# hanruihua/RDA-planner

Measured on AMD Instinct MI355X. Metric: MPC steps/sec (ADMM early stop or iter_num cap: see residuals), T=20, N_obs=200, higher is better.
Workload: dtype f64; 1 GPU; north-star: acker rectangle robot, T=20, N_obs=200 static seeded polygons, E=4, iter_num=4, iter_threshold=0.2, ro1=200; parallelism=single GPU

## Files before the change

rda_planner_amd/csrc/lammuz_device.h:

```cpp
#pragma once
#include <hip/hip_runtime.h>
#include <math.h>

#pragma clang fp contract(on)

namespace lmz {

constexpr int EMAX = 8;
constexpr int RMAX = 8;
constexpr double SIGN_TOL = 1e-12;

struct WaveLDS {
    double A[EMAX][2];
    double b[EMAX];
    double q[EMAX];
    double M[EMAX][2];
    unsigned char lamc[40];
    double vtx[28][2];
    int npv, nlv;
};
struct RobotLDS {
    double G[RMAX][2];
    double h[RMAX];
    unsigned char muc[40]; int nmv;
// ... 314 lines not shown
    if (norm2) {
        if (lane == 0) { W.lamc[0] = 1; W.lamc[1] = 2; W.lamc[2] = 0; W.npv = 0; W.nlv = 3; }
    } else {
        bool vp = false; double vx = 0, vy = 0;
        if (lane < E * (E - 1) / 2) {
            int i1, i2; decode_pair(lane, E, i1, i2);
            const double a00 = W.A[i1][0], a01 = W.A[i1][1], a10 = W.A[i2][0], a11 = W.A[i2][1];
            const double det = a00 * a11 - a01 * a10;
            if (det != 0 && det * det > 1e-24 * (a00 * a00 + a01 * a01) * (a10 * a10 + a11 * a11)) {
                const double wx = W.b[i1] * a11 - a01 * W.b[i2], wy = a00 * W.b[i2] - W.b[i1] * a10, sg = det > 0 ? 1.0 : -1.0, ad = fabs(det);
                vp = true;
                for (int k = 0; k < E; ++k) {
                    const double ak0 = W.A[k][0], ak1 = W.A[k][1], bk = W.b[k];
                    const double viol = sg * (ak0 * wx + ak1 * wy - bk * det);
                    if (viol > 1e-9 * (ad + fabs(bk) * ad + fabs(ak0 * wx) + fabs(ak1 * wy))) vp = false;
                }
                vx = wx / det; vy = wy / det;
            }
        }
        const bool vs = lane < E && (W.A[lane < E ? lane : 0][0] != 0 || W.A[lane < E ? lane : 0][1] != 0);
        const unsigned long long bp = __ballot(vp), bs = __ballot(vs), below = (1ull << lane) - 1;
        const int npv = __popcll(bp), nsv = __popcll(bs);
        if (vp) { const int k = __popcll(bp & below); W.lamc[k] = (unsigned char)(1 + E + lane); W.vtx[k][0] = vx; W.vtx[k][1] = vy; }
        if (vs) W.lamc[npv + __popcll(bs & below)] = (unsigned char)(1 + lane);
        if (lane == 0) { W.lamc[npv + nsv] = 0; W.npv = npv; W.nlv = npv + nsv + 1; }
    }
}

__device__ __forceinline__ void wave_sync()
{
    __builtin_amdgcn_fence(__ATOMIC_RELEASE, "workgroup");
    __builtin_amdgcn_wave_barrier();
    __builtin_amdgcn_fence(__ATOMIC_ACQUIRE, "workgroup");
}

__device__ __forceinline__ void prepare_wave(WaveLDS &W, const Params &P, int lane)
{
    pose_products(W, P, lane);
    build_lists(W, P.E, P.norm2, lane);
    wave_sync();
}

__device__ __forceinline__ void solve_wave(WaveLDS &W, const RobotLDS &Rb, const Params &P, int lane, Sol &best)
{
    const int nm = 1 + P.R + P.R * (P.R - 1) / 2;
    const int nlv = W.nlv, nmv = Rb.nmv;
    const int half = nlv * nmv;
    best.cost = INFINITY; best.id = 0x7fffffff;
    best.m = 0; best.H0 = 0; best.H1 = 0; best.i1 = best.i2 = best.j1 = best.j2 = -1;
    best.l1 = best.l2 = best.g1 = best.g2 = 0;
    long long tprev = P.prof ? clock64() : 0;
    auto mark = [&](int k) { if (P.prof && lane == 0) { long long now = clock64(); P.prof[k] += now - tprev; tprev = now; } };
    for (int ic = 0; ic < 2; ++ic) {
        int itn = 0;
        for (int c = lane; c < half; c += 64) {
            const int ilx = c / nmv, il = W.lamc[ilx], im = Rb.muc[c - ilx * nmv];
            Sol s;
            if (eval_candidate(W, Rb, P, il, im, ic, s)) {
                s.id = 2 * (il * nm + im) + ic;
                if (s.cost < best.cost || (s.cost == best.cost && s.id < best.id)) best = s;
            }
            mark(1 + 2 * ic + (itn < 1 ? itn : 1)); ++itn;
        }
        double bc = best.cost; int bid = best.id;
#pragma unroll
        for (int off = 32; off >= 1; off >>= 1) {
            double oc = __shfl_xor(bc, off, 64); int oid = __shfl_xor(bid, off, 64);
            if (oc < bc || (oc == bc && oid < bid)) { bc = oc; bid = oid; }
        }
        unsigned long long win = __ballot(best.id == bid);
        int src = __ffsll((long long)win) - 1;
        best.cost = __shfl(best.cost, src, 64); best.id = bid;
        best.m = __shfl(best.m, src, 64); best.H0 = __shfl(best.H0, src, 64); best.H1 = __shfl(best.H1, src, 64);
        best.i1 = __shfl(best.i1, src, 64); best.i2 = __shfl(best.i2, src, 64);
        best.j1 = __shfl(best.j1, src, 64); best.j2 = __shfl(best.j2, src, 64);
        best.l1 = __shfl(best.l1, src, 64); best.l2 = __shfl(best.l2, src, 64);
        best.g1 = __shfl(best.g1, src, 64); best.g2 = __shfl(best.g2, src, 64);
        mark(5 + ic);
        if (best.m >= 0) break;
        if (ic == 0) best.cost += 0.5 * best.m * best.m;
    }
}

template <int CTRL> __device__ __forceinline__ double dpp_mov_f64(double v)
{
    int lo = __builtin_amdgcn_update_dpp(0, __double2loint(v), CTRL, 0xf, 0xf, false);
    int hi = __builtin_amdgcn_update_dpp(0, __double2hiint(v), CTRL, 0xf, 0xf, false);
    return __hiloint2double(hi, lo);
}
template <int CTRL> __device__ __forceinline__ double dpp_mov0_f64(double v)
{
    int lo = __builtin_amdgcn_update_dpp(0, __double2loint(v), CTRL, 0xf, 0xf, true);
    int hi = __builtin_amdgcn_update_dpp(0, __double2hiint(v), CTRL, 0xf, 0xf, true);
    return __hiloint2double(hi, lo);
}
__device__ __forceinline__ double wave_max(double v)
{
    double o;
    o = dpp_mov_f64<0xB1>(v); v = o > v ? o : v;
    o = dpp_mov_f64<0x4E>(v); v = o > v ? o : v;
    o = dpp_mov_f64<0x141>(v); v = o > v ? o : v;
    o = dpp_mov_f64<0x140>(v); v = o > v ? o : v;
    o = __shfl_xor(v, 16, 64); v = o > v ? o : v;
    o = __shfl_xor(v, 32, 64); v = o > v ? o : v;
    return v;
}

__device__ __forceinline__ double row_max(double v)
{
    double o;
    o = dpp_mov_f64<0xB1>(v); v = o > v ? o : v;
    o = dpp_mov_f64<0x4E>(v); v = o > v ? o : v;
    o = dpp_mov_f64<0x141>(v); v = o > v ? o : v;
    o = dpp_mov_f64<0x140>(v); v = o > v ? o : v;
    return v;
}
template <int GW> struct Grp {
    static __device__ __forceinline__ unsigned long long ballot(bool p, int lane)
    {
        const unsigned long long b = __ballot(p);
        if (GW == 64) return b;
        return (b >> (lane & 48)) & 0xffffull;
    }
    static __device__ __forceinline__ double max(double v) { return GW == 64 ? wave_max(v) : row_max(v); }
    template <typename Tv> static __device__ __forceinline__ Tv bcast(Tv v, int src) { return __shfl(v, src, GW); }
};

__device__ __forceinline__ int support_neighbour(int c, int n, const unsigned char *cand, int ncand, int k)
{
    if (c == 0) { int seen = 0; for (int q = 0; q < ncand; ++q) { const int v = cand[q]; if (v >= 1 && v <= n) { if (seen == k) return v; ++seen; } } return -1; }
    if (c <= n) {
        if (k == 0) return 0;
        int seen = 1;
        for (int q = 0; q < ncand; ++q) {
            const int v = cand[q];
            if (v > n) { int a, b; decode_pair(v - 1 - n, n, a, b); if (a == c - 1 || b == c - 1) { if (seen == k) return v; ++seen; } }
        }
        return -1;
    }
    int a, b; decode_pair(c - 1 - n, n, a, b);
    return k == 0 ? 1 + a : (k == 1 ? 1 + b : -1);
}

template <int GW> __device__ __forceinline__ bool warm_circle(const WaveLDS &W, const RobotLDS &Rb, const Params &P, int wlane, int hint, Sol &best)
{
    const int lane = wlane & (GW - 1), R = P.R, E = P.E, nm0 = 1 + R + R * (R - 1) / 2;
    if (hint < 0) return false;
    const int il = hint / nm0, im = hint - il * nm0;
    if (il > 2) return false;
    auto certify = [&]() -> bool {
        const double na = best.i1 >= 0 ? hypot(best.l1, best.l2) : 0.0;
        if (na > 1.0 + 1e-12) return false;
        if ((best.j1 >= 0 && !(best.g1 > 1e-12)) || (best.j2 >= 0 && !(best.g2 > 1e-12))) return false;
        const double phim = (best.m < 0 ? best.m : 0.0) - P.delta;
        const double dvx = P.px - W.b[0], dvy = P.py - W.b[1], l0 = W.b[2];
        const double ut0 = P.cs * dvx + P.sn * dvy, ut1 = -P.sn * dvx + P.cs * dvy;
        const double at0 = P.cs * best.l1 + P.sn * best.l2, at1 = -P.sn * best.l1 + P.cs * best.l2;
        const double g0 = phim * ut0 + P.ro2 * best.H0, g1 = phim * ut1 + P.ro2 * best.H1, ck = phim * l0;
        const double gs = fabs(phim) * (hypot(ut0, ut1) + fabs(l0)) + P.ro2 * hypot(best.H0, best.H1);
        bool pass;
        if (!(na > 0)) pass = hypot(g0, g1) < ck * (1.0 - 1e-6);
        else {
            const double gr0 = g0 + ck * at0 / na, gr1 = g1 + ck * at1 / na;
            if (na < 1.0 - 1e-6) pass = na > 1e-6 && hypot(gr0, gr1) <= 1e-7 * gs;
            else { const double nu = -(gr0 * at0 + gr1 * at1), tz = gr1 * at0 - gr0 * at1; pass = na >= 1.0 - 1e-12 && nu > 1e-6 * gs && fabs(tz) <= 1e-7 * gs; }
        }
// ... 279 lines not shown
```

rda_planner_amd/csrc/rda_hip.hip:

```cpp
#include <hip/hip_runtime.h>
#include <cfloat>
#include <climits>
#include <cstdio>
#include <cstdlib>
#include <cstring>
#include <vector>
#include <chrono>
#include <memory>
#include <dlfcn.h>
#include "../../include/rda_hip.h"
#include "host_buf.h"
#include "lammuz_device.h"
#include "lammuz_cp_device.h"
#include "lammuz_ip_device.h"
#include "su_device.h"
#include "scene_device.h"
#include "lidar_device.h"
#include "track_device.h"
#include "rollout_device.h"

#define HIPCHK(x) do { hipError_t e_ = (x); if (e_ != hipSuccess) { \
    fprintf(stderr, "librda_hip: %s failed: %s (%s:%d)\n", #x, hipGetErrorString(e_), __FILE__, __LINE__); return RDA_ERR_HIP; } } while (0)

struct Ctrl {
// ... 444 lines not shown
    const size_t o = drow(d, n, t + 1), zi = drow(d, n, t);
    P.xi0 = d.xi[2 * o]; P.xi1 = d.xi[2 * o + 1];
    const double zeta = d.zeta[zi], dbar = d.dis[t];
    P.kappa0 = zeta - dbar; P.ro2 = d.c.ro2; P.delta = d.c.delta;
    lmz::Sol best;
    double prev = 0.0;
    if (lane < E) prev = d.lam[o * E + lane];
    else if (lane < E + R) prev = d.mu[o * R + lane - E];
    bool bad = !isfinite(P.px + P.py + P.cs + P.sn + P.xi0 + P.xi1 + P.kappa0);
    if (lane < 2 * E) bad = bad || !isfinite(W.A[lane >> 1][lane & 1]);
    if (lane < E) bad = bad || !isfinite(W.b[lane]);
    bad = __ballot(bad) != 0;
    if (bad) {
        if (lane < 2 * E) W.A[lane >> 1][lane & 1] = 0;
        if (lane < E) W.b[lane] = 0;
        P.px = P.py = P.sn = P.xi0 = P.xi1 = P.kappa0 = 0; P.cs = 1;
        lmz::wave_sync();
    }
    lmz::pose_products(W, P, lane);
    {
        const size_t oc = (size_t)n * d.nt + (d.nt > 1 ? t + 1 : 0);
        if (lane < d.oc_ls) W.lamc[lane] = d.oc_lamc[oc * d.oc_ls + lane];
        if (lane < d.oc_vs) (&W.vtx[0][0])[lane] = d.oc_vtx[oc * d.oc_vs + lane];
        if (lane == 0) { W.npv = d.oc_cnt[2 * oc]; W.nlv = d.oc_cnt[2 * oc + 1]; }
    }
    lmz::wave_sync();
    const int hpar = d.ctrl->hint_par & 1;
    if (!d.warm || !lmz::solve_wave_warm<64>(W, rb, P, lane, hint_read(d, hpar, n, t, it == 0), best)) lmz::solve_wave(W, rb, P, lane, best);
    if (lane == 0) hint_write(d, hpar, n, t, best.id >> 1);
    if (d.centre) lmz::central_normal_wave<64>(W, rb, P, lane, best);
    bad = bad || !(isfinite(best.cost) && isfinite(best.m) && isfinite(best.H0) && isfinite(best.H1));
    const int k = t * d.Nloc + nl;
    if (bad) {
        if (lane == 0) {
            store_row(d, k, failed_row(d, k));
            hint_write(d, hpar, n, t, -1);
            atomicAdd(&d.ctrl->lmz_fail, 1);
        }
        return;
    }
    const double znew = (d.c.accelerated ? 0.5 : 1.0) * (best.m > 0 ? best.m : 0.0);
    double res = 0;
    if (lane < E) {
        double v = lmz::lam_of(best, P.norm2, lane);
        res = (v - prev) * (v - prev); d.lam[o * E + lane] = v;
    } else if (lane < E + R) {
        int j = lane - E;
        double v = lmz::mu_of(best, j);
        res = (v - prev) * (v - prev); d.mu[o * R + j] = v;
    } else if (lane == E + R) {
        double old = d.z[zi];
        res = (znew - old) * (znew - old); d.z[zi] = znew;
    }
#pragma unroll
    for (int off = 32; off >= 1; off >>= 1) res += __shfl_xor(res, off, 64);
    if (lane == 0) {
        double ax = 0, ay = 0, bl = 0, mh = 0, gx = 0, gy = 0;
        for (int i = 0; i < E; ++i) {
            double v = lmz::lam_of(best, P.norm2, i);
            ax += v * W.A[i][0]; ay += v * W.A[i][1]; bl += v * W.b[i];
        }
        for (int j = 0; j < R; ++j) {
            double v = lmz::mu_of(best, j);
            mh += v * rb.h[j]; gx += v * rb.G[j][0]; gy += v * rb.G[j][1];
        }
        const double hx = gx + P.cs * ax + P.sn * ay, hy = gy - P.sn * ax + P.cs * ay;
        const double xin0 = P.xi0 + hx, xin1 = P.xi1 + hy;
        d.xi[2 * o] = xin0; d.xi[2 * o + 1] = xin1;
        const double im = ax * P.px + ay * P.py - bl - mh;
        const double zetan = zeta + im - dbar - znew;
        d.zeta[zi] = zetan;
        RowOut ro; ro.ax = ax; ro.ay = ay; ro.bl = bl; ro.c3 = mh + znew - zetan; ro.c4 = gx + xin0; ro.c5 = gy + xin1;
        ro.res = res; ro.hh = hx * hx + hy * hy;
        store_row(d, k, ro);
    }
}

__global__ __launch_bounds__(256) void k_lammuz(Dev d, int it) { lammuz_body(d, blockIdx.x, it); }

#ifdef RDA_LMZ_CLK
__device__ unsigned long long *g_lmz_clk = nullptr;
constexpr int LMZ_CLK_WORDS = 32;
__device__ int *g_lmz_faillog = nullptr;
#endif
template <int MODE = 0, bool CW = false> __device__ __forceinline__ void lammuz_body_rows(const Dev &d, const int block, const int nblocks, const int it, const Fin &fin)
{
#pragma clang fp contract(on)
    constexpr int WPB = GS / 4;
    constexpr bool LANES = CW;
    __shared__ lmz::WaveLDS wl[GS];
    __shared__ lmz::RobotLDS rb;
    __shared__ double rowv[MODE == 0 ? GS : 1][6];
    const int T = d.c.T, E = d.c.E, R = d.c.R;
#ifdef RDA_LMZ_CLK
    long long clk_prev = clock64(); const long long clk_in = clk_prev; bool clk_enum = false; const unsigned long long clk_wall_in = (unsigned long long)wall_clock64();
    unsigned long long *const clk_slot = g_lmz_clk ? g_lmz_clk + LMZ_CLK_WORDS * (size_t)(block * (GS / 4) + (threadIdx.x >> 6)) : nullptr;
    long long clk_sub = clk_prev;
#define LMZ_CLK(k) do { if (MODE == 0) { const long long now_ = clock64(); if (clk_slot && (threadIdx.x & 63) == 0) clk_slot[k] += (unsigned long long)(now_ - clk_prev); clk_prev = now_; clk_sub = now_; } } while (0)
#define LMZ_SUB(k) do { if (MODE == 0) { const long long now_ = clock64(); if (clk_slot && (threadIdx.x & 63) == 0) clk_slot[16 + (k)] += (unsigned long long)(now_ - clk_sub); clk_sub = now_; } } while (0)
#else
#define LMZ_CLK(k) do { } while (0)
#define LMZ_SUB(k) do { } while (0)
#endif
    int tb = 0, jb = 0;
    if (MODE != 2) { block_of(d, block, tb, jb); if (tb < 0) return; }
    const int lane = threadIdx.x & 63, wv = threadIdx.x >> 6, row = lane >> 4, gl = lane & 15;
    struct Early { double px, py, cs, sn, xi0, xi1, zeta, dbar, prev, vtx[4], A, b, G, h, zold, rv; int cone, src, hpar, hint, npv, nlv; unsigned char lamc[3], muc; } ey;
    if (MODE == 0) {
        const int nl0 = jb * GS + wv * 4 + row, nl = nl0 < d.Nlive ? nl0 : 0, n = d.rank * d.Nloc + nl;
        ey.src = (d.slot_src && n < d.src_used) ? d.slot_src[n] : -1;
        ey.hpar = d.ctrl->hint_par & 1;
        static_assert(64 * WPB >= 56, "one element of the robot tables per thread");
        if (LANES) { ey.muc = d.muc[(int)threadIdx.x < 40 ? threadIdx.x : 0]; ey.rv = (&d.rv[0][0])[(int)threadIdx.x < 56 ? threadIdx.x : 0]; }
    }
    if (LANES) {
        int stop = d.ctrl->stop;
        asm volatile("" : "+v"(ey.hpar), "+v"(stop));
        ey.hpar = __builtin_amdgcn_readfirstlane(ey.hpar);
        if (__builtin_amdgcn_readfirstlane(stop)) return;
    } else
    if (d.ctrl->stop) return;
    if (MODE == 2 && block * WPB >= d.ctrl->wl_count + (d.ctrl->wlc_count + 3) / 4) return;
    LMZ_CLK(0);
    if (MODE == 0) {
        const int t = tb, nl0 = jb * GS + wv * 4 + row, nl = nl0 < d.Nlive ? nl0 : 0, n = d.rank * d.Nloc + nl;
        const double *ps = d.pose + 4 * t;
        const size_t o = drow(d, n, t + 1), zi = drow(d, n, t), oc = (size_t)n * d.nt + (d.nt > 1 ? t + 1 : 0);
        ey.px = ps[0]; ey.py = ps[1]; ey.cs = ps[2]; ey.sn = ps[3];
        ey.xi0 = d.xi[2 * o]; ey.xi1 = d.xi[2 * o + 1]; ey.zeta = d.zeta[zi]; ey.dbar = d.dis[t]; ey.cone = d.cone[n];
        ey.zold = d.z[zi];
        ey.prev = *(gl < E ? &d.lam[o * E + gl] : (gl < E + R ? &d.mu[o * R + gl - E] : &d.lam[o * E]));
        {
            const size_t ao = ((size_t)n * d.nt + (d.nt > 1 ? t + 1 : 0)) * E;
            ey.A = d.A[ao * 2 + (gl < 2 * E ? gl : 0)]; ey.b = d.b[ao + (gl < E ? gl : 0)];
            ey.G = d.G[(int)threadIdx.x < 2 * R ? threadIdx.x : 0]; ey.h = d.h[(int)threadIdx.x < R ? threadIdx.x : 0];
        }
#pragma unroll
        for (int k = 0; k < 3; ++k) ey.lamc[k] = gl + 16 * k < d.oc_ls ? d.oc_lamc[oc * d.oc_ls + gl + 16 * k] : (unsigned char)0;
#pragma unroll
        for (int k = 0; k < 4; ++k) ey.vtx[k] = gl + 16 * k < d.oc_vs ? d.oc_vtx[oc * d.oc_vs + gl + 16 * k] : 0.0;
        ey.npv = d.oc_cnt[2 * oc]; ey.nlv = d.oc_cnt[2 * oc + 1];
        {
            const int key = (ey.src >= 0 && ey.src < d.src_cap) ? d.c.N + ey.src : n, tr = (it == 0 && t + 1 < T) ? t + 1 : t;
            ey.hint = d.hint[(size_t)(ey.hpar ^ 1) * d.hint_len + (size_t)tr * d.hint_stride + key];
        }
    }
    LMZ_SUB(0);
    if (MODE == 0) {
        if ((int)threadIdx.x < 2 * R) rb.G[threadIdx.x >> 1][threadIdx.x & 1] = ey.G;
        if ((int)threadIdx.x < R) rb.h[threadIdx.x] = ey.h;
    } else {
        for (int i = threadIdx.x; i < 2 * R; i += 64 * WPB) rb.G[i >> 1][i & 1] = d.G[i];
        for (int i = threadIdx.x; i < R; i += 64 * WPB) rb.h[i] = d.h[i];
    }
    if (LANES) {
        if ((int)threadIdx.x < 40) rb.muc[threadIdx.x] = ey.muc;
        if ((int)threadIdx.x < 56) (&rb.rv[0][0])[threadIdx.x] = ey.rv;
    } else {
        for (int i = threadIdx.x; i < 40; i += 64 * WPB) rb.muc[i] = d.muc[i];
        for (int i = threadIdx.x; i < 56; i += 64 * WPB) (&rb.rv[0][0])[i] = (&d.rv[0][0])[i];
    }
    if (threadIdx.x == 0) { rb.nmv = d.nmv; rb.nrv = d.nrv; }
    LMZ_SUB(1);
    const int cntP = MODE == 2 ? d.ctrl->wl_count : 1, cntC = MODE == 2 ? d.ctrl->wlc_count : 0;
    const int cnt = cntP + (cntC + 3) / 4;
    for (int base = MODE == 2 ? block * WPB : 0; base < cnt; base += MODE == 2 ? nblocks * WPB : 1) {
// ... 24 lines not shown
    __syncthreads();
    LMZ_CLK(1);
    lmz::Params P;
    P.E = E; P.R = R; P.norm2 = MODE == 0 ? ey.cone : d.cone[n];
    const double *ps = d.pose + 4 * t;
    if (MODE == 0) { P.px = ey.px; P.py = ey.py; P.cs = ey.cs; P.sn = ey.sn; }
    else { P.px = ps[0]; P.py = ps[1]; P.cs = ps[2]; P.sn = ps[3]; }
    const size_t o = drow(d, n, t + 1), zi = drow(d, n, t);
    if (MODE == 0) { P.xi0 = ey.xi0; P.xi1 = ey.xi1; } else { P.xi0 = d.xi[2 * o]; P.xi1 = d.xi[2 * o + 1]; }
    const double zeta = MODE == 0 ? ey.zeta : d.zeta[zi], dbar = MODE == 0 ? ey.dbar : d.dis[t];
    P.kappa0 = zeta - dbar; P.ro2 = d.c.ro2; P.delta = d.c.delta;
    lmz::Sol best;
    double prev = 0.0;
    if (MODE == 0) prev = gl < E + R ? ey.prev : 0.0;
    else if (gl < E) prev = d.lam[o * E + gl];
    else if (gl < E + R) prev = d.mu[o * R + gl - E];
    const double px0 = P.px, py0 = P.py;
    bool bad = !isfinite(P.px + P.py + P.cs + P.sn + P.xi0 + P.xi1 + P.kappa0);
    if (gl < 2 * E) bad = bad || !isfinite(W.A[gl >> 1][gl & 1]);
    if (gl < E) bad = bad || !isfinite(W.b[gl]);
    bad = ((__ballot(bad) >> (16 * row)) & 0xffffull) != 0;
    if (bad) {
        if (gl < 2 * E) W.A[gl >> 1][gl & 1] = 0;
        if (gl < E) W.b[gl] = 0;
        P.px = P.py = P.sn = P.xi0 = P.xi1 = P.kappa0 = 0; P.cs = 1;
    }
    lmz::wave_sync();
    lmz::pose_products(W, P, gl);
    {
        const size_t oc = (size_t)n * d.nt + (d.nt > 1 ? t + 1 : 0);
        if (MODE == 0) {
#pragma unroll
            for (int k = 0; k < 3; ++k) if (gl + 16 * k < d.oc_ls) W.lamc[gl + 16 * k] = ey.lamc[k];
#pragma unroll
            for (int k = 0; k < 4; ++k) if (gl + 16 * k < d.oc_vs) (&W.vtx[0][0])[gl + 16 * k] = ey.vtx[k];
            if (gl == 0) { W.npv = ey.npv; W.nlv = ey.nlv; }
        } else {
            for (int i = gl; i < d.oc_ls; i += 16) W.lamc[i] = d.oc_lamc[oc * d.oc_ls + i];
            for (int i = gl; i < d.oc_vs; i += 16) (&W.vtx[0][0])[i] = d.oc_vtx[oc * d.oc_vs + i];
            if (gl == 0) { W.npv = d.oc_cnt[2 * oc]; W.nlv = d.oc_cnt[2 * oc + 1]; }
        }
    }
    lmz::wave_sync();
    LMZ_CLK(2);
    const int hpar = MODE == 0 ? ey.hpar : (d.ctrl->hint_par & 1);
    const int hint_in = MODE == 0 ? ey.hint : (MODE != 2 ? hint_read(d, hpar, n, t, it == 0) : ((P.norm2 && live) ? hint_read(d, hpar, n, t, it == 0) : -1));
    bool ok = MODE != 2 && d.warm && lmz::solve_wave_warm<16>(W, rb, P, lane, hint_in, best);
    if (CW && MODE == 0 && d.warm && P.norm2 && live && !bad) ok = lmz::warm_circle<16>(W, rb, P, lane, hint_in, best);
    if (MODE == 2 && d.warm && P.norm2 && live && !bad) ok = lmz::warm_circle<16>(W, rb, P, lane, hint_in, best);
    LMZ_CLK(3);
    if (MODE != 2 && !live && !ok) {
        best.cost = 0; best.id = 0; best.m = -1; best.H0 = best.H1 = 0; best.i1 = best.i2 = best.j1 = best.j2 = -1;
        best.l1 = best.l2 = best.g1 = best.g2 = 0;
        ok = true;
    }
    unsigned long long need = __ballot(!ok);
    if (MODE == 2) {
        need = __ballot(live && !ok);
        if (!live) {
            best.cost = 0; best.id = 0; best.m = -1; best.H0 = best.H1 = 0; best.i1 = best.i2 = best.j1 = best.j2 = -1;
            best.l1 = best.l2 = best.g1 = best.g2 = 0;
        }
    }
#ifdef RDA_LMZ_STATS
    if (lane == 0) {
        const int nf = __popcll(need) >> 4;
        if (block == 0 && wv == 0) atomicAdd(&d.ctrl->lmz_stat[0], 1u);
        atomicAdd(&d.ctrl->lmz_stat[1], (unsigned)nf); atomicAdd(&d.ctrl->lmz_stat[2 + nf], 1u);
    }
#endif
    bool defer = false;
    if (MODE == 1) {
        defer = ((need >> (16 * row)) & 1) != 0 && !bad;
        if ((need >> (16 * row)) & 1) {
            best.cost = 0; best.id = 0; best.m = -1; best.H0 = best.H1 = 0; best.i1 = best.i2 = best.j1 = best.j2 = -1;
            best.l1 = best.l2 = best.g1 = best.g2 = 0;
        }
        if (defer && gl == 0 && live) {
            if (P.norm2) d.wl[d.wl_cap - 1 - atomicAdd(&d.ctrl->wlc_count, 1)] = t * GS * d.J + nl;
            else d.wl[atomicAdd(&d.ctrl->wl_count, 1)] = t * GS * d.J + nl;
        }
        need = 0;
    }
    if (MODE == 0) {
        struct Prm { int norm2; double px, py, cs, sn, xi0, xi1, kappa0; };
        __shared__ int nfail; __shared__ unsigned char flist[GS]; __shared__ Prm prm[GS]; __shared__ lmz::Sol sol[GS];
        if (threadIdx.x == 0) nfail = 0;
        __syncthreads();
        const bool mine = ((need >> (16 * row)) & 1) != 0;
        if (mine && gl == 0) {
            const int rid = wv * 4 + row; flist[atomicAdd(&nfail, 1)] = (unsigned char)rid;
            Prm &q = prm[rid]; q.norm2 = P.norm2; q.px = P.px; q.py = P.py; q.cs = P.cs; q.sn = P.sn; q.xi0 = P.xi0; q.xi1 = P.xi1; q.kappa0 = P.kappa0;
        }
        __syncthreads();
        const int nf = nfail;
        for (int i = wv; i < nf; i += WPB) {
            const int rid = flist[i];
            lmz::Params Pg;
            { const Prm &q = prm[rid]; Pg.E = E; Pg.R = R; Pg.norm2 = q.norm2; Pg.px = q.px; Pg.py = q.py; Pg.cs = q.cs; Pg.sn = q.sn; Pg.xi0 = q.xi0; Pg.xi1 = q.xi1;
              Pg.kappa0 = q.kappa0; Pg.ro2 = P.ro2; Pg.delta = P.delta; }
            lmz::Sol bg;
            lmz::solve_wave(wl[rid], rb, Pg, lane, bg);
            if (lane == 0) sol[rid] = bg;
        }
        __syncthreads();
        if (mine) best = sol[wv * 4 + row];
        need = 0;
#ifdef RDA_LMZ_CLK
        clk_enum = nf > 0;
        if (mine && gl == 0 && live && g_lmz_faillog) {
            const int k = atomicAdd(&g_lmz_faillog[0], 1);
            if (k < 200000) { g_lmz_faillog[1 + 3 * k] = hint_in; g_lmz_faillog[2 + 3 * k] = best.id >> 1; g_lmz_faillog[3 + 3 * k] = P.norm2; }
        }
#endif
    }
    LMZ_CLK(4);
    while (need) {
        const int g = (__ffsll((long long)need) - 1) >> 4;
        need &= ~(0xffffull << (16 * g));
        lmz::Params Pg;
        const int src = 16 * g;
        Pg.E = E; Pg.R = R; Pg.norm2 = __shfl(P.norm2, src, 64);
        Pg.px = __shfl(P.px, src, 64); Pg.py = __shfl(P.py, src, 64); Pg.cs = __shfl(P.cs, src, 64); Pg.sn = __shfl(P.sn, src, 64);
        Pg.xi0 = __shfl(P.xi0, src, 64); Pg.xi1 = __shfl(P.xi1, src, 64); Pg.kappa0 = __shfl(P.kappa0, src, 64);
        Pg.ro2 = P.ro2; Pg.delta = P.delta;
        lmz::Sol bg;
        lmz::solve_wave(wl[wv * 4 + g], rb, Pg, lane, bg);
        if (row == g) best = bg;
    }
    if (gl == 0 && live && !defer) {
        if (LANES) hint_write_src(d, hpar, n, t, ey.src, best.id >> 1); else hint_write(d, hpar, n, t, best.id >> 1);
    }
    LMZ_SUB(3);
#ifdef RDA_LMZ_CLK
    {
        long long cn[5]; for (int q = 0; q < 5; ++q) cn[q] = 0;
        if (d.centre) lmz::central_normal_wave<16, LANES>(W, rb, P, lane, best, cn);
        if (MODE == 0 && clk_slot && (threadIdx.x & 63) == 0) { long long pv = clk_sub; for (int q = 0; q < 5; ++q) if (cn[q]) { clk_slot[20 + q] += (unsigned long long)(cn[q] - pv); pv = cn[q]; } }
    }
#else
    if (d.centre) lmz::central_normal_wave<16, LANES>(W, rb, P, lane, best);
#endif
    LMZ_CLK(5);
    bad = bad || !(isfinite(best.cost) && isfinite(best.m) && isfinite(best.H0) && isfinite(best.H1));
    const double znew = (d.c.accelerated ? 0.5 : 1.0) * (best.m > 0 ? best.m : 0.0);
    double res = 0;
    const bool wr = live && !bad && !defer;
    if (LANES) {
        const bool isl = gl < E, ism = !isl && gl < E + R, isz = gl == E + R;
        const double vlam = lmz::lam_of(best, P.norm2, gl), vmu = lmz::mu_of(best, gl - E);
        const double v = isl ? vlam : (ism ? vmu : znew), old = isz ? ey.zold : prev;
        res = (isl || ism || isz) ? (v - old) * (v - old) : 0.0;
        double *const p = isl ? &d.lam[o * E + gl] : (ism ? &d.mu[o * R + gl - E] : &d.z[zi]);
        if (wr && gl <= E + R) *p = v;
    } else
    if (gl < E) {
        double v = lmz::lam_of(best, P.norm2, gl);
        res = (v - prev) * (v - prev); if (wr) d.lam[o * E + gl] = v;
    } else if (gl < E + R) {
        int j = gl - E;
        double v = lmz::mu_of(best, j);
        res = (v - prev) * (v - prev); if (wr) d.mu[o * R + j] = v;
    } else if (gl == E + R) {
        const double old = MODE == 0 ? ey.zold : d.z[zi];
        res = (znew - old) * (znew - old); if (wr) d.z[zi] = znew;
    }
    LMZ_SUB(9);
    if (LANES) {
        res += lmz::dpp_mov0_f64<0x128>(res);
        res += lmz::dpp_mov0_f64<0x124>(res);
        res += lmz::dpp_mov0_f64<0x4E>(res);
        res += lmz::dpp_mov0_f64<0xB1>(res);
    } else {
#pragma unroll
        for (int off = 8; off >= 1; off >>= 1) res += __shfl_xor(res, off, 16);
    }
    LMZ_SUB(10);
    double ax = 0, ay = 0, bl = 0, mh = 0, gx = 0, gy = 0;
    if (LANES) {
        const bool le = gl < E, lr = gl < R;
        const int ie = le ? E - 1 - gl : 0, je = lr ? R - 1 - gl : 0;
        const double a0r = W.A[ie][0], a1r = W.A[ie][1], bbr = W.b[ie], hhr = rb.h[je], g0r = rb.G[je][0], g1r = rb.G[je][1];
        const double vl = le ? lmz::lam_of(best, P.norm2, ie) : 0.0, vm = lr ? lmz::mu_of(best, je) : 0.0;
        const double a0 = le ? a0r : 0.0, a1 = le ? a1r : 0.0, bb = le ? bbr : 0.0, hh = lr ? hhr : 0.0, g0 = lr ? g0r : 0.0, g1 = lr ? g1r : 0.0;
        const int ns = E > R ? E : R;
        for (int s = 0; s < ns; ++s) {
            ax = vl * a0 + lmz::dpp_mov0_f64<0x101>(ax); ay = vl * a1 + lmz::dpp_mov0_f64<0x101>(ay); bl = vl * bb + lmz::dpp_mov0_f64<0x101>(bl);
            mh = vm * hh + lmz::dpp_mov0_f64<0x101>(mh); gx = vm * g0 + lmz::dpp_mov0_f64<0x101>(gx); gy = vm * g1 + lmz::dpp_mov0_f64<0x101>(gy);
        }
        LMZ_SUB(11);
    }
    if (gl == 0) {
        const int k = t * d.Nloc + nl;
        RowOut ro;
        bool have = false;
        if (live && bad) {
            ro = failed_row(d, k); have = true;
            store_row(d, k, ro);
            if (LANES) hint_write_src(d, hpar, n, t, ey.src, -1); else hint_write(d, hpar, n, t, -1);
            atomicAdd(&d.ctrl->lmz_fail, 1);
        } else if (wr) {
            if (!LANES) {
                for (int i = 0; i < E; ++i) {
                    double v = lmz::lam_of(best, P.norm2, i);
                    ax += v * W.A[i][0]; ay += v * W.A[i][1]; bl += v * W.b[i];
                }
                for (int j = 0; j < R; ++j) {
                    double v = lmz::mu_of(best, j);
                    mh += v * rb.h[j]; gx += v * rb.G[j][0]; gy += v * rb.G[j][1];
                }
                LMZ_SUB(11);
            }
            const double hx = gx + P.cs * ax + P.sn * ay, hy = gy - P.sn * ax + P.cs * ay;
            const double xin0 = P.xi0 + hx, xin1 = P.xi1 + hy;
            d.xi[2 * o] = xin0; d.xi[2 * o + 1] = xin1;
            const double im = ax * P.px + ay * P.py - bl - mh;
            const double zetan = zeta + im - dbar - znew;
            d.zeta[zi] = zetan;
            ro.ax = ax; ro.ay = ay; ro.bl = bl; ro.c3 = mh + znew - zetan; ro.c4 = gx + xin0; ro.c5 = gy + xin1;
            ro.res = res; ro.hh = hx * hx + hy * hy; have = true;
            store_row(d, k, ro);
            LMZ_SUB(12);
        }
        if (MODE == 0) {
            double *rv = rowv[wv * 4 + row];
            if (have) row_record(rv, d, ro, px0, py0);
            else { rv[0] = rv[1] = rv[2] = rv[3] = rv[4] = rv[5] = 0.0; }
        }
    }
    LMZ_CLK(6);
    if (MODE == 0) {
        __syncthreads();
        LMZ_SUB(13);
        block_partial(d, tb, jb, rowv, threadIdx.x);
        if (block == 0 && threadIdx.x == 0) d.ctrl->pose_ok = 1;
    }
    LMZ_CLK(7);
#ifdef RDA_LMZ_CLK
    if (MODE == 0 && clk_slot && (threadIdx.x & 63) == 0) {
        const unsigned long long tot = (unsigned long long)(clock64() - clk_in);
        clk_slot[8] += 1; clk_slot[9] += tot; if (tot > clk_slot[10]) clk_slot[10] = tot;
        clk_slot[13] = clk_wall_in; clk_slot[14] = (unsigned long long)wall_clock64();
        if (clk_enum) { clk_slot[11] += 1; clk_slot[12] += tot; }
    }
#endif
    }
#undef LMZ_CLK
#undef LMZ_SUB
}

__global__ __launch_bounds__(64 * GS / 4) void k_lammuz_rows(Dev d, int it, Fin fin) { warm_kernargs<sizeof(Dev) + sizeof(int) + sizeof(Fin)>(); lammuz_body_rows<0, true>(d, blockIdx.x, gridDim.x, it, fin); }
__global__ __launch_bounds__(64 * GS / 4, 2) void k_lammuz_rows_dense(Dev d, int it, Fin fin) { lammuz_body_rows<0>(d, blockIdx.x, gridDim.x, it, fin); }
__global__ __launch_bounds__(64 * GS / 4, 3) void k_lammuz_rows_fast(Dev d, int it) { lammuz_body_rows<1>(d, blockIdx.x, gridDim.x, it, Fin{}); }
__global__ __launch_bounds__(64 * GS / 4, 1) void k_lammuz_enum(Dev d, int it) { lammuz_body_rows<2>(d, blockIdx.x, gridDim.x, it, Fin{}); }

constexpr int FPB = 256 / GS;
__device__ __forceinline__ void finalize_body(const Dev &d, const int block, const int nblocks, const int it, const Fin &fin)
{
#pragma clang fp contract(on)
    __shared__ double rowv[FPB][GS][6];
    if (it >= 0 && d.ctrl->stop) return;
    const int T = d.c.T, g = threadIdx.x / GS, row = threadIdx.x % GS;
    const int B = block * FPB + g, t = B / d.J, j = B - t * d.J, nl = GS * j + row;
    double *rv = rowv[g][row];
    if (B < T * d.J && nl < d.Nlive) {
        const int k = t * d.Nloc + nl;
        RowOut ro; ro.ax = coef_arr(d, d.rank, 0)[k]; ro.ay = coef_arr(d, d.rank, 1)[k]; ro.bl = coef_arr(d, d.rank, 2)[k];
        ro.c3 = coef_arr(d, d.rank, 3)[k]; ro.c4 = coef_arr(d, d.rank, 4)[k]; ro.c5 = coef_arr(d, d.rank, 5)[k];
        ro.res = coef_arr(d, d.rank, 6)[k]; ro.hh = coef_arr(d, d.rank, 7)[k];
        row_record(rv, d, ro, d.pose[4 * t], d.pose[4 * t + 1]);
    } else { rv[0] = rv[1] = rv[2] = rv[3] = rv[4] = rv[5] = 0.0; }
    __syncthreads();
    if (B < T * d.J) block_partial(d, t, j, rowv[g], row);
    if (block == 0 && threadIdx.x == 0) d.ctrl->pose_ok = 1;
}
__global__ __launch_bounds__(256) void k_lmz_finalize(Dev d, int it, Fin fin) { finalize_body(d, blockIdx.x, gridDim.x, it, fin); }

template <int NX, int MX> __device__ __forceinline__ void lammuz_cp_body(const Dev &d, const int block)
{
    const int T = d.c.T, E = d.c.E, R = d.c.R;
    if (d.ctrl->stop) return;
    const int w = block * blockDim.x + threadIdx.x;
    if (d.obstacle_num == 0) {
        if (w < T && d.rank == (d.c.N - 1) / d.Nloc) {
            const int i = w * d.Nloc + (d.c.N - 1) % d.Nloc;
            coef_arr(d, d.rank, 0)[i] = 0; coef_arr(d, d.rank, 1)[i] = 0; coef_arr(d, d.rank, 2)[i] = 0;
            coef_arr(d, d.rank, 8)[i] = coef_arr(d, d.rank, 3)[i];
        }
        return;
    }
    if (w >= d.Nlive * T) return;
    const int nl = w % d.Nlive, t = w / d.Nlive, n = d.rank * d.Nloc + nl;
    const size_t ao = ((size_t)n * d.nt + (d.nt > 1 ? t + 1 : 0)) * E, o = drow(d, n, t + 1), zi = drow(d, n, t);
    const int k = t * d.Nloc + nl;
    double A[16], b[8];
    for (int i = 0; i < 2 * E; ++i) A[i] = d.A[ao * 2 + i];
    for (int i = 0; i < E; ++i) b[i] = d.b[ao + i];
    cpq::Problem p;
    p.E = E; p.R = R; p.cone_norm2 = d.cone[n]; p.robot_norm2 = d.c.robot_norm2; p.accelerated = d.c.accelerated;
    p.A = A; p.b = b; p.G = d.G; p.h = d.h;
    const double *ps = d.pose + 4 * t;
    p.px = ps[0]; p.py = ps[1]; p.cs = ps[2]; p.sn = ps[3];
    p.xi0 = d.xi[2 * o]; p.xi1 = d.xi[2 * o + 1];
    const double zeta = d.zeta[zi], dbar = d.dis[t];
    p.kappa0 = zeta - dbar; p.ro2 = d.c.ro2; p.mu_target = d.lmz_mu;
    bool finite_in = isfinite(p.px + p.py + p.cs + p.sn + p.xi0 + p.xi1 + p.kappa0);
    for (int i = 0; i < 2 * E; ++i) finite_in = finite_in && isfinite(A[i]);
    for (int i = 0; i < E; ++i) finite_in = finite_in && isfinite(b[i]);
    if (!finite_in) {
        store_row(d, k, failed_row(d, k));
        atomicAdd(&d.ctrl->lmz_fail, 1);
        return;
    }
    cpq::Result rs;
    {
        cpq::Solver<NX, MX> sv;
        sv.run(p, rs);
    }
    const bool fail = rs.status != 0;
    double res = 0, lam[8], mu[8], znew;
    for (int i = 0; i < E; ++i) { const double old = d.lam[o * E + i]; lam[i] = fail ? old : rs.lam[i]; res += (lam[i] - old) * (lam[i] - old); }
    for (int j = 0; j < R; ++j) { const double old = d.mu[o * R + j]; mu[j] = fail ? old : rs.mu[j]; res += (mu[j] - old) * (mu[j] - old); }
    { const double old = d.z[zi]; znew = fail ? old : rs.z; res += (znew - old) * (znew - old); }
    if (!fail) {
        for (int i = 0; i < E; ++i) d.lam[o * E + i] = lam[i];
        for (int j = 0; j < R; ++j) d.mu[o * R + j] = mu[j];
// ... 1305 lines not shown
    int rc = scan_run(H, n_beams, ranges, angle_min, angle_max, range_max, state, eps, min_samples, false, &n);
    if (rc != RDA_OK) return rc;
    rc = scene_async(H, n > 0, [&](hipStream_t st) -> int { return scan_stage(H, n, state, order, st); });
    if (rc != RDA_OK) { if (fresh) H->li = {}; return rc; }
    if (n_boxes) *n_boxes = n;
    return RDA_OK;
}

extern "C" int rda_tracked_finish(rda_handle *H, double *out_u, double *out_s, rda_info *info,
                                  double *nom_s_out, double *ref_out, int32_t *min_index, double *end_heading)
{
    if (!H || !H->tick.pending) return RDA_ERR_ARG;
    const size_t T = H->d.c.T;
    const double *in_u = H->tick.in_u;
    if (H->tick.scene_on_s2) HIPCHK(hipStreamWaitEvent(H->stream, H->ev_scene, 0));
    H->tick.pending = 0; H->tick.pending_scene = 0; H->tick.scene_on_s2 = 0;
    const StepViews v = step_views(H);
    int rc = enqueue_admm_tail(H, v.s, in_u, v.ref, v.speed, H->res.out_u(), H->res.out_s(), H->res.info());
    if (rc != RDA_OK) { (void)hipStreamSynchronize(H->stream); return rc; }
    if (nom_s_out || ref_out) {
        HIPCHK(H->step.pull(H->stream, step_speed(T)));
        HIPCHK(hipStreamSynchronize(H->stream));
    }
    rc = fetch_result(H);
    if (rc != RDA_OK) return rc;
    result_out(H->res.blk.h, H->res.h_info(), T, out_u, out_s, info);
    if (nom_s_out) memcpy(nom_s_out, H->step.h, traj_s(T) * sizeof(double));
    if (ref_out) memcpy(ref_out, H->step.h + step_ref(T), traj_s(T) * sizeof(double));
    if (min_index) *min_index = H->res.h_track()->min_index;
    if (end_heading) *end_heading = H->res.h_track()->end_heading;
    return RDA_OK;
}

extern "C" int rda_step_tracked(rda_handle *H, const double *state, double ref_speed, int cur_index, double threshold, int ind_range,
                                const double *nom_u, double *out_u, double *out_s, rda_info *info,
                                double *nom_s_out, double *ref_out, int32_t *min_index, double *end_heading)
{
    if (!H || !state || !out_u || !out_s) return RDA_ERR_ARG;
    int rc = rda_tracked_begin(H, state, ref_speed, cur_index, threshold, ind_range, nom_u);
    if (rc != RDA_OK) return rc;
    return rda_tracked_finish(H, out_u, out_s, info, nom_s_out, ref_out, min_index, end_heading);
}

extern "C" int rda_upload_trace(rda_handle *H, int K, const double *nom_s, const double *nom_u, const double *ref_s, const double *ref_speed)
{
    if (!H || K < 1 || !nom_s || !nom_u || !ref_s || !ref_speed) return RDA_ERR_ARG;
    const size_t ns = traj_s(H->d.c.T), nu = traj_u(H->d.c.T);
    TraceSet t;
    if (t.alloc((size_t)K, ns, nu)) return RDA_ERR_HIP;
    HIPCHK(hipMemcpy(t.s, nom_s, K * ns * sizeof(double), hipMemcpyHostToDevice));
    HIPCHK(hipMemcpy(t.u, nom_u, K * nu * sizeof(double), hipMemcpyHostToDevice));
    HIPCHK(hipMemcpy(t.ref, ref_s, K * ns * sizeof(double), hipMemcpyHostToDevice));
    HIPCHK(hipMemcpy(t.speed, ref_speed, K * sizeof(double), hipMemcpyHostToDevice));
    H->trace = std::move(t);
    return RDA_OK;
}

extern "C" int rda_enqueue_step(rda_handle *H, int k)
{
    if (!H || k < 0 || k >= H->trace.K) return RDA_ERR_ARG;
    const size_t ns = traj_s(H->d.c.T), nu = traj_u(H->d.c.T);
    return enqueue_admm(H, H->trace.s + k * ns, H->trace.u + k * nu, H->trace.ref + k * ns, H->trace.speed + k,
                        H->trace.out_u + k * nu, H->trace.out_s + k * ns, H->trace.info + k);
}

extern "C" int rda_enqueue_range(rda_handle *H, int k0, int k1)
{
    if (!H || k0 < 0 || k1 > H->trace.K || k0 > k1) return RDA_ERR_ARG;
    for (int k = k0; k < k1; ++k) { int rc = rda_enqueue_step(H, k); if (rc != RDA_OK) return rc; }
    return RDA_OK;
}

#ifdef RDA_LMZ_CLK
extern "C" int rda_debug_lmz_clk(rda_handle *H, unsigned long long *out, int max_waves)
{
    static unsigned long long *buf = nullptr; static int cap = 0;
    static hbuf::Group &keep = *new hbuf::Group;
    HIPCHK(hipStreamSynchronize(H->stream));
    if (!buf) {
        hbuf::Group g; unsigned long long *b;
        if (g.dev(&b, (size_t)max_waves * LMZ_CLK_WORDS)) return RDA_ERR_HIP;
        HIPCHK(hipMemcpyToSymbol(HIP_SYMBOL(g_lmz_clk), &b, sizeof(b)));
        keep.d.push_back(std::move(g.d[0])); buf = b; cap = max_waves;
        return RDA_OK;
    }
    if (max_waves < 0) {
        static int *flog = nullptr;
        if (!flog) {
            hbuf::Group g; int *f;
            if (g.dev(&f, 1 + 3 * 200000)) return RDA_ERR_HIP;
            HIPCHK(hipMemcpyToSymbol(HIP_SYMBOL(g_lmz_faillog), &f, sizeof(f)));
            keep.d.push_back(std::move(g.d[0])); flog = f;
            return RDA_OK;
        }
        HIPCHK(hipMemcpy(out, flog, (1 + 3 * 200000) * sizeof(int), hipMemcpyDeviceToHost));
        HIPCHK(hipMemset(flog, 0, sizeof(int)));
        return RDA_OK;
    }
    if (max_waves > cap) return RDA_ERR_ARG;
    HIPCHK(hipMemcpy(out, buf, (size_t)max_waves * LMZ_CLK_WORDS * sizeof(unsigned long long), hipMemcpyDeviceToHost));
    HIPCHK(hipMemset(buf, 0, (size_t)cap * LMZ_CLK_WORDS * sizeof(unsigned long long)));
    return RDA_OK;
}
#endif
#ifdef RDA_LMZ_STATS
extern "C" int rda_debug_lmz_stats(rda_handle *H, unsigned *out)
{
    HIPCHK(hipStreamSynchronize(H->stream));
    HIPCHK(hipMemcpy(out, (char *)H->d.ctrl + offsetof(Ctrl, lmz_stat), 8 * sizeof(unsigned), hipMemcpyDeviceToHost));
    return RDA_OK;
}
#endif
extern "C" int rda_sync(rda_handle *H) { if (!H) return RDA_ERR_ARG; HIPCHK(hipStreamSynchronize(H->stream)); H->tick.pending_scene = 0; return RDA_OK; }

extern "C" int rda_fetch_result(rda_handle *H, int k, double *out_u, double *out_s, rda_info *info)
{
    if (!H || k < 0 || k >= H->trace.K) return RDA_ERR_ARG;
    const size_t ns = traj_s(H->d.c.T), nu = traj_u(H->d.c.T);
    HIPCHK(hipStreamSynchronize(H->stream));
    if (out_u) HIPCHK(hipMemcpy(out_u, H->trace.out_u + k * nu, nu * sizeof(double), hipMemcpyDeviceToHost));
    if (out_s) HIPCHK(hipMemcpy(out_s, H->trace.out_s + k * ns, ns * sizeof(double), hipMemcpyDeviceToHost));
    if (info) HIPCHK(hipMemcpy(info, H->trace.info + k, sizeof(rda_info), hipMemcpyDeviceToHost));
    return RDA_OK;
}

extern "C" int rda_timing_reset(rda_handle *H, int enable)
{
    if (!H) return RDA_ERR_ARG;
    HIPCHK(hipStreamSynchronize(H->stream));
    HIPCHK(hipStreamSynchronize(H->stream2));
    H->timing = enable; H->ev_used[0] = H->ev_used[1] = H->ev_used[2] = H->ev_used[3] = 0;
    return RDA_OK;
}
extern "C" int rda_timing_read(rda_handle *H, int which, double *total_ms, int *launches)
{
    if (!H || which < 0 || which > 3) return RDA_ERR_ARG;
    HIPCHK(hipStreamSynchronize(which == 3 ? H->stream2 : H->stream));
    double tot = 0; int n = 0;
    for (size_t i = 0; i + 1 < H->ev_used[which]; i += 2) {
        float ms = 0; HIPCHK(hipEventElapsedTime(&ms, H->ev[which][i], H->ev[which][i + 1]));
        tot += ms; ++n;
    }
    if (total_ms) *total_ms = tot;
    if (launches) *launches = n;
    return RDA_OK;
}

extern "C" int rda_timing_launches(rda_handle *H, int which, double *ms_out, int cap, int *launches)
{
    if (!H || which < 0 || which > 3 || (cap > 0 && !ms_out)) return RDA_ERR_ARG;
    HIPCHK(hipStreamSynchronize(which == 3 ? H->stream2 : H->stream));
    int n = 0;
    for (size_t i = 0; i + 1 < H->ev_used[which]; i += 2, ++n) {
        if (n >= cap) continue;
        float ms = 0; HIPCHK(hipEventElapsedTime(&ms, H->ev[which][i], H->ev[which][i + 1]));
        ms_out[n] = ms;
    }
    if (launches) *launches = n;
    return RDA_OK;
}

static void tr_to_host(const std::vector<double> &dev, double *host, size_t N, size_t TT, size_t W)
{
    for (size_t n = 0; n < N; ++n) for (size_t t = 0; t < TT; ++t) memcpy(host + (n * TT + t) * W, dev.data() + (t * N + n) * W, W * sizeof(double));
}
static void tr_to_dev(const double *host, std::vector<double> &dev, size_t N, size_t TT, size_t W)
// ... 1979 lines not shown
```

Measured before the change: 4303 steps/s.

## Split fallback candidate enumeration of each failed row across both waves

```diff
diff --git a/rda_planner_amd/csrc/lammuz_device.h b/rda_planner_amd/csrc/lammuz_device.h
--- a/rda_planner_amd/csrc/lammuz_device.h
+++ b/rda_planner_amd/csrc/lammuz_device.h
@@ -420,6 +420,45 @@
     }
 }
 
+__device__ __forceinline__ void solve_wave_pair(WaveLDS &W, const RobotLDS &Rb, const Params &P, int lane, int wv, Sol *xch, Sol &best)
+{
+    const int nm = 1 + P.R + P.R * (P.R - 1) / 2;
+    const int nlv = W.nlv, nmv = Rb.nmv;
+    const int half = nlv * nmv;
+    best.cost = INFINITY; best.id = 0x7fffffff;
+    best.m = 0; best.H0 = 0; best.H1 = 0; best.i1 = best.i2 = best.j1 = best.j2 = -1;
+    best.l1 = best.l2 = best.g1 = best.g2 = 0;
+    const int cut = (P.norm2 ? 1 : W.npv) * nmv;
+    const int c_lo = wv ? cut : 0, c_hi = wv ? half : cut;
+    for (int ic = 0; ic < 2; ++ic) {
+        for (int c = c_lo + lane; c < c_hi; c += 64) {
+            const int ilx = c / nmv, il = W.lamc[ilx], im = Rb.muc[c - ilx * nmv];
+            Sol s;
+            if (eval_candidate(W, Rb, P, il, im, ic, s)) {
+                s.id = 2 * (il * nm + im) + ic;
+                if (s.cost < best.cost || (s.cost == best.cost && s.id < best.id)) best = s;
+            }
+        }
+        double bc = best.cost; int bid = best.id;
+#pragma unroll
+        for (int off = 32; off >= 1; off >>= 1) {
+            double oc = __shfl_xor(bc, off, 64); int oid = __shfl_xor(bid, off, 64);
+            if (oc < bc || (oc == bc && oid < bid)) { bc = oc; bid = oid; }
+        }
+        unsigned long long win = __ballot(best.id == bid);
+        int src = __ffsll((long long)win) - 1;
+        Sol *const own = xch + 2 * ic + wv;
+        if (lane == src) *own = best;
+        __syncthreads();
+        const Sol *const oth = xch + 2 * ic + (wv ^ 1);
+        const double c0 = own->cost, c1 = oth->cost; const int i0 = own->id, i1 = oth->id;
+        const Sol *const w = (c1 < c0 || (c1 == c0 && i1 < i0)) ? oth : own;
+        best = *w;
+        if (__builtin_amdgcn_readfirstlane((int)(best.m >= 0))) break;
+        if (ic == 0) best.cost += 0.5 * best.m * best.m;
+    }
+}
+
 template <int CTRL> __device__ __forceinline__ double dpp_mov_f64(double v)
 {
     int lo = __builtin_amdgcn_update_dpp(0, __double2loint(v), CTRL, 0xf, 0xf, false);
diff --git a/rda_planner_amd/csrc/rda_hip.hip b/rda_planner_amd/csrc/rda_hip.hip
--- a/rda_planner_amd/csrc/rda_hip.hip
+++ b/rda_planner_amd/csrc/rda_hip.hip
@@ -550,6 +550,8 @@
 __device__ unsigned long long *g_lmz_clk = nullptr;
 constexpr int LMZ_CLK_WORDS = 32;
 __device__ int *g_lmz_faillog = nullptr;
+constexpr int LMZ_SPAN_CAP = 4096;
+__device__ unsigned long long *g_lmz_span = nullptr;
 #endif
 template <int MODE = 0, bool CW = false> __device__ __forceinline__ void lammuz_body_rows(const Dev &d, const int block, const int nblocks, const int it, const Fin &fin)
 {
@@ -740,6 +742,38 @@
         }
         need = 0;
     }
+    if (MODE == 0 && CW) {
+        static_assert(WPB == 2, "lmz::solve_wave_pair: the two waves of the workgroup");
+        struct Prm { int norm2; double px, py, cs, sn, xi0, xi1, kappa0; };
+        __shared__ unsigned char needw[WPB]; __shared__ Prm prm[GS]; __shared__ lmz::Sol xch[2][4];
+        const bool mine = ((need >> (16 * row)) & 1) != 0;
+        if (mine && gl == 0) {
+            Prm &q = prm[wv * 4 + row]; q.norm2 = P.norm2; q.px = P.px; q.py = P.py; q.cs = P.cs; q.sn = P.sn; q.xi0 = P.xi0; q.xi1 = P.xi1; q.kappa0 = P.kappa0;
+        }
+        if (lane == 0) needw[wv] = (unsigned char)((need & 1) | ((need >> 15) & 2) | ((need >> 30) & 4) | ((need >> 45) & 8));
+        __syncthreads();
+        unsigned mask = __builtin_amdgcn_readfirstlane((unsigned)needw[0] | ((unsigned)needw[1] << 4));
+#ifdef RDA_LMZ_CLK
+        clk_enum = mask != 0;
+#endif
+        for (int k = 0; mask; ++k) {
+            const int rid = __ffs((int)mask) - 1;
+            mask &= mask - 1;
+            lmz::Params Pg;
+            { const Prm &q = prm[rid]; Pg.E = E; Pg.R = R; Pg.norm2 = q.norm2; Pg.px = q.px; Pg.py = q.py; Pg.cs = q.cs; Pg.sn = q.sn; Pg.xi0 = q.xi0; Pg.xi1 = q.xi1;
+              Pg.kappa0 = q.kappa0; Pg.ro2 = P.ro2; Pg.delta = P.delta; }
+            lmz::Sol bg;
+            lmz::solve_wave_pair(wl[rid], rb, Pg, lane, wv, xch[k & 1], bg);
+            if (wv * 4 + row == rid) best = bg;
+        }
+        need = 0;
+#ifdef RDA_LMZ_CLK
+        if (mine && gl == 0 && live && g_lmz_faillog) {
+            const int k = atomicAdd(&g_lmz_faillog[0], 1);
+            if (k < 200000) { g_lmz_faillog[1 + 3 * k] = hint_in; g_lmz_faillog[2 + 3 * k] = best.id >> 1; g_lmz_faillog[3 + 3 * k] = P.norm2; }
+        }
+#endif
+    } else
     if (MODE == 0) {
         struct Prm { int norm2; double px, py, cs, sn, xi0, xi1, kappa0; };
         __shared__ int nfail; __shared__ unsigned char flist[GS]; __shared__ Prm prm[GS]; __shared__ lmz::Sol sol[GS];
@@ -896,10 +930,15 @@
     LMZ_CLK(7);
 #ifdef RDA_LMZ_CLK
     if (MODE == 0 && clk_slot && (threadIdx.x & 63) == 0) {
-        const unsigned long long tot = (unsigned long long)(clock64() - clk_in);
+        const unsigned long long tot = (unsigned long long)(clock64() - clk_in), wall_out = (unsigned long long)wall_clock64();
+        const unsigned long long li = clk_slot[8];
         clk_slot[8] += 1; clk_slot[9] += tot; if (tot > clk_slot[10]) clk_slot[10] = tot;
-        clk_slot[13] = clk_wall_in; clk_slot[14] = (unsigned long long)wall_clock64();
+        clk_slot[13] = clk_wall_in; clk_slot[14] = wall_out;
         if (clk_enum) { clk_slot[11] += 1; clk_slot[12] += tot; }
+        if (g_lmz_span && li < (unsigned long long)LMZ_SPAN_CAP) {
+            atomicMax(&g_lmz_span[3 * li], ~clk_wall_in); atomicMax(&g_lmz_span[3 * li + 1], wall_out);
+            if (clk_enum) atomicMax(&g_lmz_span[3 * li + 2], 1ull);
+        }
     }
 #endif
     }
@@ -2371,6 +2410,20 @@
         if (g.dev(&b, (size_t)max_waves * LMZ_CLK_WORDS)) return RDA_ERR_HIP;
         HIPCHK(hipMemcpyToSymbol(HIP_SYMBOL(g_lmz_clk), &b, sizeof(b)));
         keep.d.push_back(std::move(g.d[0])); buf = b; cap = max_waves;
+        return RDA_OK;
+    }
+    if (max_waves == -2) {
+        static unsigned long long *span = nullptr;
+        if (!span) {
+            hbuf::Group g; unsigned long long *s;
+            if (g.dev(&s, (size_t)3 * LMZ_SPAN_CAP)) return RDA_ERR_HIP;
+            HIPCHK(hipMemset(s, 0, (size_t)3 * LMZ_SPAN_CAP * sizeof(unsigned long long)));
+            HIPCHK(hipMemcpyToSymbol(HIP_SYMBOL(g_lmz_span), &s, sizeof(s)));
+            keep.d.push_back(std::move(g.d[0])); span = s;
+            return RDA_OK;
+        }
+        HIPCHK(hipMemcpy(out, span, (size_t)3 * LMZ_SPAN_CAP * sizeof(unsigned long long), hipMemcpyDeviceToHost));
+        HIPCHK(hipMemset(span, 0, (size_t)3 * LMZ_SPAN_CAP * sizeof(unsigned long long)));
         return RDA_OK;
     }
     if (max_waves < 0) {
```

Result: slower. 4235 steps/s (-1.6%).
